# LiZhuoHong/SegLand

Hardware: AMD Instinct MI355X
Metric: 512x512 tiles/sec fwd+bwd PSPNet-POP (higher is better)
Workload: dtype bf16; 1 GPU; PSPNet-POP resnet50 bf16, batch 16/GPU, 512x512, 8 logit channels, train_base.py loop body (fwd+loss+bwd+clip+AdamW x2), 1 x MI355X; global_batch=16, parallelism=dp1

## Files before the change

include/segland_hip_debug.h:

```cpp
#ifndef SEGLAND_HIP_DEBUG_H
#define SEGLAND_HIP_DEBUG_H
#include "segland_hip.h"
#ifdef __cplusplus
extern "C" {
#endif

void sl_debug_reset(void);

void sl_debug_conv_affine(int on);
void sl_debug_conv_p9(int on);
void sl_debug_conv_p9_lean(int on);
void sl_debug_conv_p8_k1(int on);
void sl_debug_conv_ring192(int on);
void sl_debug_conv_ringn64(int on);
void sl_debug_conv_rows_small(int on);
void sl_debug_ppm_fact_walk(int on);
void sl_debug_conv_parity(int on);
void sl_debug_ring_small_k(int k);
void sl_debug_ring64_max_tiles(int tiles);
void sl_debug_wgrad3(int on);
void sl_debug_wgrad_bias(int on);
void sl_debug_wgrad_tr(int on);
void sl_debug_wgrad_pair_min(int rows);
void sl_debug_attn_valu(int v);
void sl_debug_ce_tiled(int on);

void sl_debug_p8_trace(void* buf);
void sl_debug_wgrad_trace(void* buf);
void sl_debug_wgrad3_trace(void* buf);
void sl_debug_attn_trace(void* buf);

int sl_debug_wgrad3_plan(const SlConvDesc* d, int* out);

#ifdef __cplusplus
}
#endif
#endif
```

segland_amd/csrc/api.cpp:

```cpp
#include <stdarg.h>
#include <stdio.h>
#include <mutex>
#include <unordered_map>
#include "common.h"

static thread_local char g_err[512] = "";

void sl_set_error(const char* fmt, ...) {
  va_list ap;
  va_start(ap, fmt);
  vsnprintf(g_err, sizeof(g_err), fmt, ap);
  va_end(ap);
}

extern "C" int sl_version(void) { return 100; }
extern "C" const char* sl_last_error_string(void) { return g_err; }

__attribute__((visibility("hidden"))) int sl_lds_opt_in(const char* name, const void* kernel, size_t lds_bytes) {
  static std::mutex mu;
  static std::unordered_map<const void*, size_t> granted;
  std::lock_guard<std::mutex> lock(mu);
  size_t& have = granted[kernel];
  if (lds_bytes <= have) return 0;
  const hipError_t e = hipFuncSetAttribute(kernel, hipFuncAttributeMaxDynamicSharedMemorySize, (int)lds_bytes);
  if (e != hipSuccess) {
    sl_set_error("%s: opt-in to %zu bytes of dynamic LDS refused: %s", name, lds_bytes, hipGetErrorString(e));
    return (int)e;
  }
  have = lds_bytes;
  return 0;
}

extern "C" int sl_hip_clear_error(void) { return (int)hipGetLastError(); }

#include "../../include/segland_hip_debug.h"
SlDebugState g_sl_debug;
extern "C" void sl_debug_reset(void) { g_sl_debug = SlDebugState(); }
extern "C" void sl_debug_conv_affine(int v) { g_sl_debug.conv_affine = v ? 1 : 0; }
extern "C" void sl_debug_conv_p9(int v) { g_sl_debug.conv_p9 = (v & 1) ? 1 : 0; }
extern "C" void sl_debug_conv_p9_lean(int v) { g_sl_debug.conv_p9_lean = v ? 1 : 0; }
extern "C" void sl_debug_conv_p8_k1(int v) { g_sl_debug.conv_p8_k1 = v ? 1 : 0; }
extern "C" void sl_debug_conv_ring192(int v) { g_sl_debug.conv_ring192 = v ? 1 : 0; }
extern "C" void sl_debug_conv_ringn64(int v) { g_sl_debug.conv_ringn64 = v ? 1 : 0; }
extern "C" void sl_debug_conv_rows_small(int v) { g_sl_debug.conv_rows_small = v ? 1 : 0; }
extern "C" void sl_debug_conv_parity(int v) { g_sl_debug.conv_parity = v ? 1 : 0; }
extern "C" void sl_debug_ppm_fact_walk(int v) { g_sl_debug.ppm_fact_walk = v ? 1 : 0; }
extern "C" void sl_debug_ring64_max_tiles(int v) { g_sl_debug.ring64_max_tiles = v; }
extern "C" void sl_debug_ring_small_k(int v) { g_sl_debug.ring_small_k = v; }
extern "C" void sl_debug_wgrad3(int v) { g_sl_debug.wgrad3 = v ? 1 : 0; }
extern "C" void sl_debug_wgrad_bias(int v) { g_sl_debug.wgrad_bias = v ? 1 : 0; }
extern "C" void sl_debug_wgrad_tr(int v) { g_sl_debug.wgrad_tr = v ? 1 : 0; }
extern "C" void sl_debug_wgrad_pair_min(int rows) { g_sl_debug.wgrad_pair_min_rows = rows; }
extern "C" void sl_debug_attn_valu(int v) { g_sl_debug.attn_valu = v; }
extern "C" void sl_debug_ce_tiled(int v) { g_sl_debug.ce_tiled = v ? 1 : 0; }
extern "C" void sl_debug_p8_trace(void* buf) { g_sl_debug.p8_trace = (unsigned long long*)buf; }
extern "C" void sl_debug_wgrad_trace(void* buf) { g_sl_debug.wgrad_trace = (unsigned long long*)buf; }
extern "C" void sl_debug_wgrad3_trace(void* buf) { g_sl_debug.wgrad3_trace = (unsigned long long*)buf; }
extern "C" void sl_debug_attn_trace(void* buf) { g_sl_debug.attn_trace = (unsigned long long*)buf; }
```

segland_amd/csrc/common.h:

```cpp
#pragma once
#include <hip/hip_runtime.h>
#include <stdint.h>
#include <stdio.h>
#include "../../include/segland_hip.h"

typedef unsigned short bf16_t;

typedef __attribute__((ext_vector_type(8))) __bf16 bf16x8_t;
typedef __attribute__((ext_vector_type(16))) float f32x16_t;
typedef __attribute__((ext_vector_type(4))) float f32x4_t;

__device__ __forceinline__ float bf2f(bf16_t v) { return __uint_as_float(((unsigned)v) << 16); }
__device__ __forceinline__ bf16_t f2bf(float f) {
  return __builtin_bit_cast(bf16_t, (__bf16)f);
}

template <typename T> __device__ __forceinline__ float to_f(T v);
template <> __device__ __forceinline__ float to_f<float>(float v) { return v; }
template <> __device__ __forceinline__ float to_f<bf16_t>(bf16_t v) { return bf2f(v); }
template <typename T> __device__ __forceinline__ T from_f(float v);
template <> __device__ __forceinline__ float from_f<float>(float v) { return v; }
template <> __device__ __forceinline__ bf16_t from_f<bf16_t>(float v) { return f2bf(v); }

template <typename T> struct Vec16 { static constexpr int N = 16 / sizeof(T); };

template <typename T> __device__ __forceinline__ void unpack16(const uint4& v, float* out);
template <> __device__ __forceinline__ void unpack16<float>(const uint4& v, float* out) {
  out[0] = __uint_as_float(v.x); out[1] = __uint_as_float(v.y); out[2] = __uint_as_float(v.z); out[3] = __uint_as_float(v.w);
}
template <> __device__ __forceinline__ void unpack16<bf16_t>(const uint4& v, float* out) {
  out[0] = __uint_as_float(v.x << 16); out[1] = __uint_as_float(v.x & 0xffff0000u);
  out[2] = __uint_as_float(v.y << 16); out[3] = __uint_as_float(v.y & 0xffff0000u);
  out[4] = __uint_as_float(v.z << 16); out[5] = __uint_as_float(v.z & 0xffff0000u);
  out[6] = __uint_as_float(v.w << 16); out[7] = __uint_as_float(v.w & 0xffff0000u);
}
template <typename T> __device__ __forceinline__ uint4 pack16(const float* in);
template <> __device__ __forceinline__ uint4 pack16<float>(const float* in) {
  return make_uint4(__float_as_uint(in[0]), __float_as_uint(in[1]), __float_as_uint(in[2]), __float_as_uint(in[3]));
}
template <> __device__ __forceinline__ uint4 pack16<bf16_t>(const float* in) {
  typedef __attribute__((ext_vector_type(2))) __bf16 bf16x2_t;
  typedef __attribute__((ext_vector_type(2))) float f32x2_t;
  uint4 r;
  r.x = __builtin_bit_cast(unsigned, __builtin_convertvector((f32x2_t){in[0], in[1]}, bf16x2_t));
  r.y = __builtin_bit_cast(unsigned, __builtin_convertvector((f32x2_t){in[2], in[3]}, bf16x2_t));
  r.z = __builtin_bit_cast(unsigned, __builtin_convertvector((f32x2_t){in[4], in[5]}, bf16x2_t));
  r.w = __builtin_bit_cast(unsigned, __builtin_convertvector((f32x2_t){in[6], in[7]}, bf16x2_t));
  return r;
}

__device__ __forceinline__ float sl_erf_as(float x) {
  const float ax = fabsf(x);
  const float t = __builtin_amdgcn_rcpf(fmaf(0.3275911f, ax, 1.f));
  float p = fmaf(1.061405429f, t, -1.453152027f);
  p = fmaf(p, t, 1.421413741f); p = fmaf(p, t, -0.284496736f); p = fmaf(p, t, 0.254829592f);
  const float r = fmaf(-p * t, __expf(-ax * ax), 1.f);
  return copysignf(r, x);
}
template <typename T> __device__ __forceinline__ float sl_gelu(float x) {
  if constexpr (sizeof(T) == 4) return 0.5f * x * (1.f + erff(x * 0.70710678118654752440f));
  else return 0.5f * x * (1.f + sl_erf_as(x * 0.70710678118654752440f));
}

template <typename T> __device__ __forceinline__ float sl_gelu_grad(float x) {
  const float pdf = 0.39894228040143267794f * __expf(-0.5f * x * x);
  float cdf;
  if constexpr (sizeof(T) == 4) cdf = 0.5f * (1.f + erff(x * 0.70710678118654752440f));
  else cdf = 0.5f * (1.f + sl_erf_as(x * 0.70710678118654752440f));
  return cdf + x * pdf;
}

__device__ __forceinline__ float wave_sum(float v) {
#pragma unroll
  for (int o = 32; o > 0; o >>= 1) v += __shfl_xor(v, o, 64);
  return v;
}

void sl_set_error(const char* fmt, ...);

struct SlDebugState {
  int conv_affine = 1;
  int conv_p9 = 1;
  int conv_p9_lean = 1;
  int conv_p8_k1 = 1;
  int conv_ring192 = 1;
  int conv_ringn64 = 1;
  int conv_rows_small = 1;
  int ppm_fact_walk = 1;
  int conv_parity = 1;
  int ring_small_k = 128;
  long long ring64_max_tiles = 256;
  int wgrad3 = 1;
  int wgrad_bias = 1;
  int wgrad_tr = 1;
  long long wgrad_pair_min_rows = 0;
  int attn_valu = -1;
  int ce_tiled = 1;
  unsigned long long* p8_trace = nullptr;
  unsigned long long* wgrad_trace = nullptr;
  unsigned long long* wgrad3_trace = nullptr;
  unsigned long long* attn_trace = nullptr;
};
extern SlDebugState g_sl_debug;
#define SL_REQUIRE(cond, ...)            \
  do {                                   \
    if (!(cond)) {                       \
      sl_set_error(__VA_ARGS__);         \
      return SL_EINVAL;                  \
    }                                    \
  } while (0)
#define SL_TRY(expr)                     \
  do {                                   \
    const int rc__ = (expr);             \
    if (rc__) return rc__;               \
  } while (0)

int sl_lds_opt_in(const char* name, const void* kernel, size_t lds_bytes);

template <typename T> struct sl_as_is { typedef T type; };

template <typename... Args>
static inline int sl_launch(const char* name, void (*kernel)(Args...), dim3 grid, dim3 block, size_t lds_bytes, hipStream_t stream, typename sl_as_is<Args>::type... args) {
  if (lds_bytes > 64 * 1024) SL_TRY(sl_lds_opt_in(name, (const void*)kernel, lds_bytes));
  hipLaunchKernelGGL(kernel, grid, block, lds_bytes, stream, args...);
  const hipError_t e = hipGetLastError();
  if (e != hipSuccess) {
    sl_set_error("%s: %s", name, hipGetErrorString(e));
    return (int)e;
  }
  return 0;
}

template <typename F>
static inline int sl_by_dtype(int dtype, const char* entry, F&& f) {
  if (dtype == SL_BF16) return f(bf16_t());
  if (dtype == SL_F32) return f(float());
  sl_set_error("%s: bad dtype", entry);
  return SL_EINVAL;
}

__host__ __device__ static inline int cdiv(long long a, long long b) { return (int)((a + b - 1) / b); }

template <typename T>
__device__ __forceinline__ void sl_colsum_rows_block(const T* __restrict__ x, long long rows, int C, long long rows_per_block, float* __restrict__ part, int block, float* red) {
  constexpr int V = Vec16<T>::N;
  const int nvec = C / V;
  const int tpr = nvec < 256 ? nvec : 256, rpb = 256 / tpr;
  const int tr = threadIdx.x / tpr, tc = threadIdx.x % tpr;
  const long long r0 = (long long)block * rows_per_block, r1 = r0 + rows_per_block < rows ? r0 + rows_per_block : rows;
  for (int vc = tc; vc < nvec; vc += tpr) {
    float s[V];
#pragma unroll
    for (int k = 0; k < V; ++k) s[k] = 0.f;
    if (tr < rpb) {
      long long r = r0 + tr;
      for (; r + 3 * rpb < r1; r += 4 * rpb) {
        uint4 q[4];
#pragma unroll
        for (int u = 0; u < 4; ++u) q[u] = ((const uint4*)x)[(size_t)(r + u * rpb) * nvec + vc];
#pragma unroll
        for (int u = 0; u < 4; ++u) {
          float v[V];
          unpack16<T>(q[u], v);
#pragma unroll
          for (int k = 0; k < V; ++k) s[k] += v[k];
        }
      }
      for (; r < r1; r += rpb) {
        float v[V];
        unpack16<T>(((const uint4*)x)[(size_t)r * nvec + vc], v);
#pragma unroll
        for (int k = 0; k < V; ++k) s[k] += v[k];
      }
    }
    __syncthreads();
#pragma unroll
    for (int k = 0; k < V; ++k) red[threadIdx.x * V + k] = s[k];
    __syncthreads();
    if (tr == 0) {
#pragma unroll
      for (int k = 0; k < V; ++k) {
        float a = 0.f;
        for (int j = 0; j < rpb; ++j) a += red[(j * tpr + tc) * V + k];
        part[(size_t)block * C + vc * V + k] = a;
      }
    }
  }
}


inline long long sl_colsum_rows_chunk(long long rows, int C, int esize) {
  const int nvec = C * esize / 16, tpr = nvec < 256 ? nvec : 256, rpb = 256 / tpr;
  long long rpblk = (long long)rpb * 16;
  const long long cap = 2048;
  if ((rows + rpblk - 1) / rpblk > cap) rpblk = ((rows + cap - 1) / cap + rpb - 1) / rpb * rpb;
  return rpblk;
}
```

segland_amd/csrc/conv_gemm_sk.hip:

```cpp
#include "conv_gemm_common.h"

namespace {

using slconv::C64_T;
constexpr int C64_PW = C64_T + 2, C64_PITCH = 144;
constexpr int C64_WFRAG = 2 * 36 * 64 * 16;
constexpr int C64_LDS = C64_WFRAG + C64_PW * C64_PW * C64_PITCH + 4 * 2 * 64 * (int)sizeof(float);
__global__ __launch_bounds__(256) void conv_c64k3_kernel(ConvGemmParams p, int ntiles) {
  extern __shared__ __attribute__((aligned(16))) unsigned char smem[];
  uint4* wl = (uint4*)smem;
  unsigned char* patch = smem + C64_WFRAG;
  float* red = (float*)(patch + C64_PW * C64_PW * C64_PITCH);
  const int tid = threadIdx.x, lane = tid & 63, wave = tid >> 6, l31 = lane & 31, fh = lane >> 5;
  const int H = p.Hs, W = p.Ws;
  const int tx = cdiv(W, C64_T), ty = cdiv(H, C64_T);
  const bf16_t* src = (const bf16_t*)p.src1;
  for (int e = tid; e < 2 * 36 * 64; e += 256) {
    const int ln = e & 63, ks = (e >> 6) % 36, nb = (e >> 6) / 36;
    wl[e] = *(const uint4*)((const bf16_t*)p.wt + ((size_t)(nb * 32 + (ln & 31)) * 9 + (ks >> 2)) * 64 + (ks & 3) * 16 + (ln >> 5) * 8);
  }
  constexpr int NCH = C64_PW * C64_PW * 8, CPT = (NCH + 255) / 256;
  uint4 stage[CPT];
  auto fetch = [&](int tile) {
    int blk = tile;
    const int bx = blk % tx; blk /= tx;
    const int by = blk % ty; const int b = blk / ty;
#pragma unroll
    for (int u = 0; u < CPT; ++u) {
      const int e = tid + u * 256;
      uint4 v = make_uint4(0, 0, 0, 0);
      if (e < NCH) {
        const int ch8 = e & 7, pp = e >> 3, py = pp / C64_PW, px = pp - py * C64_PW;
        const int iy = by * C64_T - 1 + py, ix = bx * C64_T - 1 + px;
        if ((unsigned)iy < (unsigned)H && (unsigned)ix < (unsigned)W) v = *(const uint4*)(src + ((size_t)(b * H + iy) * W + ix) * 64 + ch8 * 8);
      }
      stage[u] = v;
    }
  };
  int pbase[2];
#pragma unroll
  for (int rb = 0; rb < 2; ++rb) {
    const int pidx = wave * 64 + rb * 32 + l31;
    pbase[rb] = ((pidx >> 4) * C64_PW + (pidx & 15)) * C64_PITCH + fh * 16;
  }
  if ((int)blockIdx.x < ntiles) fetch(blockIdx.x);
  for (int tile = blockIdx.x; tile < ntiles; tile += gridDim.x) {
    int blk = tile;
    const int bx = blk % tx; blk /= tx;
    const int by = blk % ty; const int b = blk / ty;
#pragma unroll
    for (int u = 0; u < CPT; ++u) {
      const int e = tid + u * 256;
      if (e < NCH) *(uint4*)(patch + (e >> 3) * C64_PITCH + (e & 7) * 16) = stage[u];
    }
    __syncthreads();
    if (tile + (int)gridDim.x < ntiles) fetch(tile + gridDim.x);
    f32x16_t acc[2][2];
#pragma unroll
    for (int rb = 0; rb < 2; ++rb)
#pragma unroll
      for (int nb = 0; nb < 2; ++nb)
#pragma unroll
        for (int r = 0; r < 16; ++r) acc[rb][nb][r] = 0.f;
#pragma unroll 4
    for (int ks = 0; ks < 36; ++ks) {
      int tap = ks >> 2;
      if (p.mode) tap = 8 - tap;
      const int ky = tap / 3, kx = tap - 3 * ky;
      const int toff = (ky * C64_PW + kx) * C64_PITCH + (ks & 3) * 32;
      const uint4 w0 = wl[(0 * 36 + ks) * 64 + lane], w1 = wl[(1 * 36 + ks) * 64 + lane];
#pragma unroll
      for (int rb = 0; rb < 2; ++rb) {
        const uint4 a = *(const uint4*)(patch + pbase[rb] + toff);
        acc[rb][0] = __builtin_amdgcn_mfma_f32_32x32x16_bf16(__builtin_bit_cast(bf16x8_t, w0), __builtin_bit_cast(bf16x8_t, a), acc[rb][0], 0, 0, 0);
        acc[rb][1] = __builtin_amdgcn_mfma_f32_32x32x16_bf16(__builtin_bit_cast(bf16x8_t, w1), __builtin_bit_cast(bf16x8_t, a), acc[rb][1], 0, 0, 0);
      }
    }
    __syncthreads();
    unsigned char* outt = patch;
#pragma unroll
    for (int rb = 0; rb < 2; ++rb) {
      const int pidx = wave * 64 + rb * 32 + l31;
#pragma unroll
      for (int nb = 0; nb < 2; ++nb)
#pragma unroll
        for (int q = 0; q < 4; ++q) {
          uint2 pk;
          pk.x = (unsigned)f2bf(acc[rb][nb][4 * q + 0]) | ((unsigned)f2bf(acc[rb][nb][4 * q + 1]) << 16);
          pk.y = (unsigned)f2bf(acc[rb][nb][4 * q + 2]) | ((unsigned)f2bf(acc[rb][nb][4 * q + 3]) << 16);
          *(uint2*)(outt + pidx * C64_PITCH + (nb * 32 + 8 * q + 4 * fh) * 2) = pk;
        }
    }
    __syncthreads();
    bf16_t* out = (bf16_t*)p.out;
    float sa[8], sq[8];
#pragma unroll
    for (int c = 0; c < 8; ++c) { sa[c] = 0.f; sq[c] = 0.f; }
    if (p.gate) {
      float mu[8], is[8];
#pragma unroll
      for (int c = 0; c < 8; ++c) { mu[c] = p.bn_mean[(tid & 7) * 8 + c]; is[c] = p.bn_invstd[(tid & 7) * 8 + c]; }
      uint4 xv[8]; unsigned bits[8];
#pragma unroll
      for (int u = 0; u < 8; ++u) {
        const int e = tid + u * 256, pidx = e >> 3, ch8 = e & 7;
        const int oy = by * C64_T + (pidx >> 4), ox = bx * C64_T + (pidx & 15);
        const bool in = oy < H && ox < W;
        const size_t pix = in ? (size_t)(b * H + oy) * W + ox : 0;
        xv[u] = *(const uint4*)((const bf16_t*)p.bn_x + pix * 64 + ch8 * 8);
        bits[u] = p.gate[pix * 8 + ch8];
      }
#pragma unroll
      for (int u = 0; u < 8; ++u) {
        const int e = tid + u * 256, pidx = e >> 3, ch8 = e & 7;
        const int oy = by * C64_T + (pidx >> 4), ox = bx * C64_T + (pidx & 15);
        if (oy < H && ox < W) {
          uint4 v = *(const uint4*)(outt + pidx * C64_PITCH + ch8 * 16);
          const unsigned bb = bits[u];
          v.x &= ((unsigned)__builtin_amdgcn_sbfe(bb, 0, 1) & 0xffffu) | ((unsigned)__builtin_amdgcn_sbfe(bb, 1, 1) & 0xffff0000u);
          v.y &= ((unsigned)__builtin_amdgcn_sbfe(bb, 2, 1) & 0xffffu) | ((unsigned)__builtin_amdgcn_sbfe(bb, 3, 1) & 0xffff0000u);
          v.z &= ((unsigned)__builtin_amdgcn_sbfe(bb, 4, 1) & 0xffffu) | ((unsigned)__builtin_amdgcn_sbfe(bb, 5, 1) & 0xffff0000u);
          v.w &= ((unsigned)__builtin_amdgcn_sbfe(bb, 6, 1) & 0xffffu) | ((unsigned)__builtin_amdgcn_sbfe(bb, 7, 1) & 0xffff0000u);
          st16(out + ((size_t)(b * H + oy) * W + ox) * 64 + ch8 * 8, v);
          const unsigned wv[4] = {v.x, v.y, v.z, v.w}, xw[4] = {xv[u].x, xv[u].y, xv[u].z, xv[u].w};
#pragma unroll
          for (int c = 0; c < 4; ++c) {
            const float lo = __uint_as_float(wv[c] << 16), hi = __uint_as_float(wv[c] & 0xffff0000u);
            const float xl = __uint_as_float(xw[c] << 16), xh = __uint_as_float(xw[c] & 0xffff0000u);
            sa[2 * c] += lo; sq[2 * c] += lo * ((xl - mu[2 * c]) * is[2 * c]);
            sa[2 * c + 1] += hi; sq[2 * c + 1] += hi * ((xh - mu[2 * c + 1]) * is[2 * c + 1]);
          }
        }
      }
    } else
#pragma unroll
    for (int u = 0; u < 8; ++u) {
      const int e = tid + u * 256;
      const int pidx = e >> 3, ch8 = e & 7;
      const int oy = by * C64_T + (pidx >> 4), ox = bx * C64_T + (pidx & 15);
      if (oy < H && ox < W) {
        const uint4 v = *(const uint4*)(outt + pidx * C64_PITCH + ch8 * 16);
        st16(out + ((size_t)(b * H + oy) * W + ox) * 64 + ch8 * 8, v);
        if (p.stat_partial) {
          const unsigned wv[4] = {v.x, v.y, v.z, v.w};
#pragma unroll
          for (int c = 0; c < 4; ++c) {
            const float lo = __uint_as_float(wv[c] << 16), hi = __uint_as_float(wv[c] & 0xffff0000u);
            sa[2 * c] += lo; sq[2 * c] += lo * lo; sa[2 * c + 1] += hi; sq[2 * c + 1] += hi * hi;
          }
        }
      }
    }
    if (p.stat_partial) {
#pragma unroll
      for (int c = 0; c < 8; ++c)
#pragma unroll
        for (int o = 8; o < 64; o <<= 1) { sa[c] += __shfl_xor(sa[c], o); sq[c] += __shfl_xor(sq[c], o); }
      if (lane < 8) {
#pragma unroll
        for (int c = 0; c < 8; ++c) { red[(wave * 2 + 0) * 64 + lane * 8 + c] = sa[c]; red[(wave * 2 + 1) * 64 + lane * 8 + c] = sq[c]; }
      }
      __syncthreads();
      if (tid < 128) {
        const int which = tid >> 6, ch = tid & 63;
        p.stat_partial[((size_t)tile * 2 + which) * 64 + ch] = red[(0 * 2 + which) * 64 + ch] + red[(1 * 2 + which) * 64 + ch] + red[(2 * 2 + which) * 64 + ch] + red[(3 * 2 + which) * 64 + ch];
      }
    }
    __syncthreads();
  }
}

}

bool slconv::c64k3_shape(int dtype, int KH, int KW, int stride, int pad, int dil, int Cin, int C1, int Cout, long long M) {
  return dtype == SL_BF16 && KH == 3 && KW == 3 && stride == 1 && pad == 1 && dil == 1 && Cin == 64 && C1 == 64 && Cout == 64 && M >= 65536;
}

int slconv::launch_c64k3(ConvGemmParams& p, hipStream_t st) {
  const int ntiles = p.B * cdiv(p.Hs, C64_T) * cdiv(p.Ws, C64_T);
  return sl_launch("conv_c64k3_kernel", conv_c64k3_kernel, dim3(ntiles < 256 ? ntiles : 256), dim3(256), C64_LDS, st, p, ntiles);
}

namespace {
template <int KS> struct SkGeom {
  static constexpr int RB = KS * 32;
  static constexpr int BSTEP = 64 * RB;
  static constexpr int STG_PITCH = 144, STG_WAVE = 32 * STG_PITCH;
  static constexpr int OFF_STG = 2 * BSTEP, OFF_RED = OFF_STG + 8 * STG_WAVE;
  static constexpr int LDS = OFF_RED + 2 * 8 * 3 * 64 * (int)sizeof(float);
};
template <int KS> __device__ __forceinline__ int sk_swz(int row) { return KS == 16 ? (row & 31) : (KS == 8 ? (row & 15) : ((row >> 1) & 7)); }
__device__ __forceinline__ float sk_sum_8_16_32(float v) {
  typedef __attribute__((ext_vector_type(2))) unsigned u32x2_t;
  v += __int_as_float(__builtin_amdgcn_update_dpp(0, __float_as_int(v), 0x128, 0xf, 0xf, false));
  u32x2_t r = __builtin_amdgcn_permlane16_swap(__float_as_uint(v), __float_as_uint(v), false, false);
  v = __uint_as_float(r.x) + __uint_as_float(r.y);
  r = __builtin_amdgcn_permlane32_swap(__float_as_uint(v), __float_as_uint(v), false, false);
  return __uint_as_float(r.x) + __uint_as_float(r.y);
}

#ifndef SL_SK_ABL
#define SL_SK_ABL 0
#endif
template <int KS, int MODE, bool SKEW>
__global__ __launch_bounds__(512, (KS == 4 && MODE != 5) ? 4 : 2) void conv_gemm_sk_kernel(ConvGemmParams p) {
  using G = SkGeom<KS>;
  using T = bf16_t;
  typedef __attribute__((ext_vector_type(2))) __bf16 bf16x2_t;
  typedef __attribute__((ext_vector_type(2))) float f32x2_t;
  extern __shared__ __attribute__((aligned(16))) unsigned char smem[];
  const int tid = threadIdx.x, lane = tid & 63;
  const int wave = __builtin_amdgcn_readfirstlane(tid >> 6);
  const int grp = wave >> 2;
  const int l31 = lane & 31, fh = lane >> 5;
  const int bm = blockIdx.x;
  const int NS = p.N / 64;
  const unsigned lds_base = __builtin_amdgcn_readfirstlane(lds_addr_of(smem));
  constexpr int NWI = SKEW ? 4 : 8, NI = 2 * KS / NWI, LPR = 2 * KS, RPI = 64 / LPR;
  const int iw = SKEW ? (wave & 3) : wave;
  const bool issuer = !SKEW || grp == 0;
  const unsigned char* bsrc[NI];
#pragma unroll
  for (int j = 0; j < NI; ++j) {
    const int row = (iw * NI + j) * RPI + lane / LPR, pos = lane % LPR;
    bsrc[j] = (const unsigned char*)p.wt + (size_t)row * G::RB + ((pos ^ sk_swz<KS>(row)) << 4);
  }
  auto issueB = [&](int s, int buf) {
#pragma unroll
    for (int j = 0; j < NI; ++j) glds16_asm(bsrc[j] + (size_t)s * G::BSTEP, lds_base + buf * G::BSTEP + (iw * NI + j) * 1024);
  };
  auto colstep = [&](int i) { return i; };
  if (issuer) issueB(colstep(0), 0);
  uint4 a[KS];
  {
    const unsigned char* arow = (const unsigned char*)p.src1 + ((size_t)bm * 256 + wave * 32 + l31) * G::RB + fh * 16;
#pragma unroll
    for (int ks = 0; ks < KS; ++ks) a[ks] = *(const uint4*)(arow + ks * 32);
  }
  int foff[KS];
  {
    const int x = sk_swz<KS>(l31);
#pragma unroll
    for (int ks = 0; ks < KS; ++ks) foff[ks] = l31 * G::RB + (((2 * ks + fh) ^ x) << 4);
  }
  unsigned char* stg = smem + G::OFF_STG + wave * G::STG_WAVE;
  float* red = (float*)(smem + G::OFF_RED);
  const int srow = lane >> 3, sch = lane & 7;
  const size_t orow = (size_t)bm * 256 + wave * 32 + srow;
  long long arow[4];
  if constexpr (MODE == 2 || MODE == 5) {
#pragma unroll
    for (int it = 0; it < 4; ++it) {
      const long long m = (long long)orow + it * 8;
      arow[it] = m;
      if (p.addend_half) {
        const int hw = p.Hd * p.Wd;
        const int b = (int)(m / hw), rem = (int)(m - (long long)b * hw), y = rem / p.Wd, x = rem - y * p.Wd;
        arow[it] = ((y | x) & 1) ? -1 : ((long long)b * (p.Hd >> 1) + (y >> 1)) * (p.Wd >> 1) + (x >> 1);
      }
    }
  }
  uint4 addv[4], cxv[4], cxv2[4];
  float bmu[8], bis[8], bmu2[8], bis2[8];
  const bool dual = MODE == 5 && p.bn_x2 != nullptr;
  const int mpitch = p.N / 8 + 16;
  unsigned char* msk = smem + (MODE == 5 ? G::LDS : G::OFF_RED);
  if ((MODE == 2 && p.addend_mask) || MODE == 5) {
    const int cpr = p.N / 128;
    const unsigned char* src = (MODE == 5 ? p.gate : p.addend_mask) + (size_t)bm * 256 * (p.N / 8);
    for (int e = tid; e < 256 * cpr; e += 512) {
      const int row = e / cpr, c = e - row * cpr;
      *(uint4*)(msk + row * mpitch + c * 16) = *(const uint4*)(src + (size_t)e * 16);
    }
  }

  auto multiply = [&](int i) {
    const int cur = i & 1, s = colstep(i);
    if (issuer && i + 1 < NS) issueB(colstep(i + 1), cur ^ 1);
    if constexpr (MODE == 2 || MODE == 5) {
      const int ncol = s * 64 + sch * 8;
#pragma unroll
      for (int it = 0; it < 4; ++it) addv[it] = (arow[it] >= 0 && !(SL_SK_ABL & 2)) ? *(const uint4*)((const T*)p.addend + arow[it] * p.N + ncol) : make_uint4(0, 0, 0, 0);
      if constexpr (MODE == 5) {
#pragma unroll
        for (int it = 0; it < 4; ++it) cxv[it] = (SL_SK_ABL & 2) ? make_uint4(0, 0, 0, 0) : *(const uint4*)((const T*)p.bn_x + (orow + it * 8) * p.N + ncol);
#pragma unroll
        for (int e = 0; e < 8; ++e) { bmu[e] = p.bn_mean[ncol + e]; bis[e] = p.bn_invstd[ncol + e]; }
        if (dual) {
#pragma unroll
          for (int it = 0; it < 4; ++it) cxv2[it] = *(const uint4*)((const T*)p.bn_x2 + (orow + it * 8) * p.N + ncol);
#pragma unroll
          for (int e = 0; e < 8; ++e) { bmu2[e] = p.bn_mean2[ncol + e]; bis2[e] = p.bn_invstd2[ncol + e]; }
        }
      }
    }
    f32x16_t acc[2];
#pragma unroll
    for (int j = 0; j < 2; ++j)
#pragma unroll
      for (int r = 0; r < 16; ++r) acc[j][r] = 0.f;
    const unsigned char* bb = smem + cur * G::BSTEP;
#pragma unroll
    for (int ks = 0; ks < KS; ++ks) {
      const uint4 b0 = *(const uint4*)(bb + foff[ks]), b1 = *(const uint4*)(bb + 32 * G::RB + foff[ks]);
      if constexpr (!(SL_SK_ABL & 8)) {
      Mma<T>::run(b0, a[ks], acc[0]);
      Mma<T>::run(b1, a[ks], acc[1]);
      } else { acc[0][0] += __uint_as_float(b0.x); acc[1][0] += __uint_as_float(b1.x); }
    }
#pragma unroll
    for (int j = 0; j < 2; ++j)
#pragma unroll
      for (int q = 0; q < 4; ++q) {
        uint2 v;
        v.x = __builtin_bit_cast(unsigned, __builtin_convertvector((f32x2_t){acc[j][4 * q + 0], acc[j][4 * q + 1]}, bf16x2_t));
        v.y = __builtin_bit_cast(unsigned, __builtin_convertvector((f32x2_t){acc[j][4 * q + 2], acc[j][4 * q + 3]}, bf16x2_t));
        *(uint2*)(stg + l31 * G::STG_PITCH + 64 * j + 16 * q + 8 * fh) = v;
      }
  };

  auto store = [&](int i) {
    const int cur = i & 1, s = colstep(i);
    const int ncol = s * 64 + sch * 8;
    wait_vmcnt<0>();
    float sa[8], sq[8], sq2[8];
#pragma unroll
    for (int e = 0; e < 8; ++e) { sa[e] = 0.f; sq[e] = 0.f; sq2[e] = 0.f; }
#pragma unroll
    for (int it = 0; it < 4; ++it) {
      const uint4 raw = *(const uint4*)(stg + (it * 8 + srow) * G::STG_PITCH + sch * 16);
      T* o = (T*)p.out + (orow + it * 8) * p.N + ncol;
      if constexpr (MODE == 1) {
        st16(o, raw);
        if (p.stat_partial) {
          const unsigned w[4] = {raw.x, raw.y, raw.z, raw.w};
#pragma unroll
          for (int c = 0; c < 4; ++c) {
            const float lo = __uint_as_float(w[c] << 16), hi = __uint_as_float(w[c] & 0xffff0000u);
            sa[2 * c] += lo; sq[2 * c] += lo * lo; sa[2 * c + 1] += hi; sq[2 * c + 1] += hi * hi;
          }
        }
      } else {
        uint4 ad = addv[it];
        if (MODE == 2 && p.addend_mask) {
          const unsigned b = msk[(wave * 32 + it * 8 + srow) * mpitch + s * 8 + sch];
          ad.x &= ((unsigned)__builtin_amdgcn_sbfe(b, 0, 1) & 0xffffu) | ((unsigned)__builtin_amdgcn_sbfe(b, 1, 1) & 0xffff0000u);
          ad.y &= ((unsigned)__builtin_amdgcn_sbfe(b, 2, 1) & 0xffffu) | ((unsigned)__builtin_amdgcn_sbfe(b, 3, 1) & 0xffff0000u);
          ad.z &= ((unsigned)__builtin_amdgcn_sbfe(b, 4, 1) & 0xffffu) | ((unsigned)__builtin_amdgcn_sbfe(b, 5, 1) & 0xffff0000u);
          ad.w &= ((unsigned)__builtin_amdgcn_sbfe(b, 6, 1) & 0xffffu) | ((unsigned)__builtin_amdgcn_sbfe(b, 7, 1) & 0xffff0000u);
        }
        const unsigned rw[4] = {raw.x, raw.y, raw.z, raw.w}, aw[4] = {ad.x, ad.y, ad.z, ad.w};
        unsigned ow[4];
#pragma unroll
        for (int c = 0; c < 4; ++c) {
          const f32x2_t v = (f32x2_t){__uint_as_float(rw[c] << 16) + __uint_as_float(aw[c] << 16), __uint_as_float(rw[c] & 0xffff0000u) + __uint_as_float(aw[c] & 0xffff0000u)};
          ow[c] = __builtin_bit_cast(unsigned, __builtin_convertvector(v, bf16x2_t));
        }
        if constexpr (MODE == 5) {
          const unsigned b = msk[(wave * 32 + it * 8 + srow) * mpitch + s * 8 + sch];
          ow[0] &= ((unsigned)__builtin_amdgcn_sbfe(b, 0, 1) & 0xffffu) | ((unsigned)__builtin_amdgcn_sbfe(b, 1, 1) & 0xffff0000u);
          ow[1] &= ((unsigned)__builtin_amdgcn_sbfe(b, 2, 1) & 0xffffu) | ((unsigned)__builtin_amdgcn_sbfe(b, 3, 1) & 0xffff0000u);
          ow[2] &= ((unsigned)__builtin_amdgcn_sbfe(b, 4, 1) & 0xffffu) | ((unsigned)__builtin_amdgcn_sbfe(b, 5, 1) & 0xffff0000u);
          ow[3] &= ((unsigned)__builtin_amdgcn_sbfe(b, 6, 1) & 0xffffu) | ((unsigned)__builtin_amdgcn_sbfe(b, 7, 1) & 0xffff0000u);
          const unsigned xw[4] = {cxv[it].x, cxv[it].y, cxv[it].z, cxv[it].w};
#pragma unroll
          for (int c = 0; c < 4; ++c) {
            if constexpr (SL_SK_ABL & 4) { sa[2 * c] += __uint_as_float(ow[c] ^ xw[c]); continue; }
            const float glo = __uint_as_float(ow[c] << 16), ghi = __uint_as_float(ow[c] & 0xffff0000u);
            const float xlo = __uint_as_float(xw[c] << 16), xhi = __uint_as_float(xw[c] & 0xffff0000u);
            sa[2 * c] += glo; sq[2 * c] += glo * ((xlo - bmu[2 * c]) * bis[2 * c]);
            sa[2 * c + 1] += ghi; sq[2 * c + 1] += ghi * ((xhi - bmu[2 * c + 1]) * bis[2 * c + 1]);
          }
          if (dual) {
            const unsigned yw[4] = {cxv2[it].x, cxv2[it].y, cxv2[it].z, cxv2[it].w};
#pragma unroll
            for (int c = 0; c < 4; ++c) {
              const float glo = __uint_as_float(ow[c] << 16), ghi = __uint_as_float(ow[c] & 0xffff0000u);
              const float ylo = __uint_as_float(yw[c] << 16), yhi = __uint_as_float(yw[c] & 0xffff0000u);
              sq2[2 * c] += glo * ((ylo - bmu2[2 * c]) * bis2[2 * c]);
              sq2[2 * c + 1] += ghi * ((yhi - bmu2[2 * c + 1]) * bis2[2 * c + 1]);
            }
          }
        }
        if constexpr (SL_SK_ABL & 1) { if (ow[0] == 0x12345678u && ow[1] == 0x9abcdef0u) st16(o, make_uint4(ow[0], ow[1], ow[2], ow[3])); }
        else st16(o, make_uint4(ow[0], ow[1], ow[2], ow[3]));
      }
    }
    if ((MODE == 1 || MODE == 5) && p.stat_partial) {
#pragma unroll
      for (int e = 0; e < 8; ++e) { sa[e] = sk_sum_8_16_32(sa[e]); sq[e] = sk_sum_8_16_32(sq[e]); }
      if (dual) {
#pragma unroll
        for (int e = 0; e < 8; ++e) sq2[e] = sk_sum_8_16_32(sq2[e]);
      }
      if (lane < 8) {
        float* r0 = red + ((cur * 8 + wave) * 3) * 64 + sch * 8;
        *(float4*)(r0) = make_float4(sa[0], sa[1], sa[2], sa[3]); *(float4*)(r0 + 4) = make_float4(sa[4], sa[5], sa[6], sa[7]);
        *(float4*)(r0 + 64) = make_float4(sq[0], sq[1], sq[2], sq[3]); *(float4*)(r0 + 68) = make_float4(sq[4], sq[5], sq[6], sq[7]);
        if (dual) { *(float4*)(r0 + 128) = make_float4(sq2[0], sq2[1], sq2[2], sq2[3]); *(float4*)(r0 + 132) = make_float4(sq2[4], sq2[5], sq2[6], sq2[7]); }
      }
    }
  };
  auto finalize = [&](int i, int t0) {
    const int s = colstep(i);
    if ((MODE == 1 || MODE == 5) && p.stat_partial && tid >= t0 && tid < t0 + (dual ? 192 : 128)) {
      const int which = (tid - t0) >> 6, col = tid & 63;
      const float* r0 = red + ((i & 1) * 24 + which) * 64 + col;
      float t = 0.f;
#pragma unroll
      for (int k = 0; k < 8; ++k) t += r0[k * 192];
      if (which < 2) p.stat_partial[((size_t)bm * 2 + which) * p.N + s * 64 + col] = t;
      if (dual && which != 1) p.stat_partial2[((size_t)bm * 2 + (which >> 1)) * p.N + s * 64 + col] = t;
    }
  };

  auto bar = [&]() { asm volatile("s_waitcnt lgkmcnt(0)\n\ts_barrier" ::: "memory"); };
  wait_vmcnt<0>();
  bar();
  if constexpr (!SKEW) {
#pragma unroll 1
    for (int s = 0; s < NS; ++s) {
      multiply(s);
      store(s);
      bar();
      finalize(s, 0);
    }
  } else if (grp == 0) {
#pragma unroll 1
    for (int s = 0; s < NS; ++s) {
      multiply(s);
      bar();
      store(s);
      bar();
    }
    bar();
  } else {
    bar();
#pragma unroll 1
    for (int s = 0; s < NS; ++s) {
      multiply(s);
      bar();
      store(s);
      bar();
      finalize(s, 256);
    }
  }
}

}

bool slconv::sk_shape(int dtype, int KH, int KW, int stride, int pad, int Cin, int C1, int N, long long M) {
  return dtype == SL_BF16 && KH == 1 && KW == 1 && stride == 1 && pad == 0 && C1 == Cin && (Cin == 64 || Cin == 128 || Cin == 256) &&
         N % 64 == 0 && M >= 65536 && M % 256 == 0;
}

namespace {
template <int KS, int MODE, bool SKEW>
int launch_sk_t(ConvGemmParams& p, hipStream_t st) {
  const int lds = MODE == 5 ? SkGeom<KS>::LDS + 256 * (p.N / 8 + 16)
                            : (MODE == 2 && p.addend_mask ? SkGeom<KS>::OFF_RED + 256 * (p.N / 8 + 16) : SkGeom<KS>::LDS);
  return sl_launch("conv_gemm_sk_kernel", conv_gemm_sk_kernel<KS, MODE, SKEW>, dim3(p.M / 256), dim3(512), lds, st, p);
}
template <int MODE, bool SKEW>
int launch_sk_k(ConvGemmParams& p, hipStream_t st) {
  return p.C1 == 256 ? launch_sk_t<16, MODE, SKEW>(p, st) : (p.C1 == 128 ? launch_sk_t<8, MODE, SKEW>(p, st) : launch_sk_t<4, MODE, SKEW>(p, st));
}
}

int slconv::launch_sk(ConvGemmParams& p, hipStream_t st) {
  constexpr int skew = 1;
  p.gridM = p.M / 256; p.gridN = 1;
  if (p.gate) return launch_sk_k<5, false>(p, st);
  if (p.addend) return (skew & 4) ? launch_sk_k<2, true>(p, st) : launch_sk_k<2, false>(p, st);
  return (skew & (p.stat_partial ? 1 : 2)) ? launch_sk_k<1, true>(p, st) : launch_sk_k<1, false>(p, st);
}
```

Before: 699.4 tiles/s.

## Prefetch addend and BN inputs two column steps ahead in sk conv GEMM

```diff
diff --git a/include/segland_hip_debug.h b/include/segland_hip_debug.h
--- a/include/segland_hip_debug.h
+++ b/include/segland_hip_debug.h
@@ -11,6 +11,7 @@
 void sl_debug_conv_p9(int on);
 void sl_debug_conv_p9_lean(int on);
 void sl_debug_conv_p8_k1(int on);
+void sl_debug_conv_sk_ahead(int on);
 void sl_debug_conv_ring192(int on);
 void sl_debug_conv_ringn64(int on);
 void sl_debug_conv_rows_small(int on);
diff --git a/segland_amd/csrc/api.cpp b/segland_amd/csrc/api.cpp
--- a/segland_amd/csrc/api.cpp
+++ b/segland_amd/csrc/api.cpp
@@ -40,6 +40,7 @@
 extern "C" void sl_debug_conv_p9(int v) { g_sl_debug.conv_p9 = (v & 1) ? 1 : 0; }
 extern "C" void sl_debug_conv_p9_lean(int v) { g_sl_debug.conv_p9_lean = v ? 1 : 0; }
 extern "C" void sl_debug_conv_p8_k1(int v) { g_sl_debug.conv_p8_k1 = v ? 1 : 0; }
+extern "C" void sl_debug_conv_sk_ahead(int v) { g_sl_debug.conv_sk_ahead = v ? 1 : 0; }
 extern "C" void sl_debug_conv_ring192(int v) { g_sl_debug.conv_ring192 = v ? 1 : 0; }
 extern "C" void sl_debug_conv_ringn64(int v) { g_sl_debug.conv_ringn64 = v ? 1 : 0; }
 extern "C" void sl_debug_conv_rows_small(int v) { g_sl_debug.conv_rows_small = v ? 1 : 0; }
diff --git a/segland_amd/csrc/common.h b/segland_amd/csrc/common.h
--- a/segland_amd/csrc/common.h
+++ b/segland_amd/csrc/common.h
@@ -83,6 +83,7 @@
   int conv_p9 = 1;
   int conv_p9_lean = 1;
   int conv_p8_k1 = 1;
+  int conv_sk_ahead = 1;
   int conv_ring192 = 1;
   int conv_ringn64 = 1;
   int conv_rows_small = 1;
diff --git a/segland_amd/csrc/conv_gemm_sk.hip b/segland_amd/csrc/conv_gemm_sk.hip
--- a/segland_amd/csrc/conv_gemm_sk.hip
+++ b/segland_amd/csrc/conv_gemm_sk.hip
@@ -199,10 +199,23 @@
   return __uint_as_float(r.x) + __uint_as_float(r.y);
 }
 
+__device__ __forceinline__ void sk_wait_vm0() {
+  asm volatile("" ::: "memory");
+  __builtin_amdgcn_s_waitcnt(0x0f70);
+  asm volatile("" ::: "memory");
+}
+template <int V> struct SkPf { static constexpr int value = V; };
+__device__ __forceinline__ uint4 sk_take(const uint4& v) {
+  uint4 r;
+  asm volatile("v_mov_b32 %0, %4\n\tv_mov_b32 %1, %5\n\tv_mov_b32 %2, %6\n\tv_mov_b32 %3, %7" : "=&v"(r.x), "=&v"(r.y), "=&v"(r.z), "=&v"(r.w) : "v"(v.x), "v"(v.y), "v"(v.z), "v"(v.w));
+  return r;
+}
+__device__ __forceinline__ unsigned sk_fresh(unsigned v) { asm volatile("" : "+v"(v)); return v; }
+
 #ifndef SL_SK_ABL
 #define SL_SK_ABL 0
 #endif
-template <int KS, int MODE, bool SKEW>
+template <int KS, int MODE, bool SKEW, bool AHEAD>
 __global__ __launch_bounds__(512, (KS == 4 && MODE != 5) ? 4 : 2) void conv_gemm_sk_kernel(ConvGemmParams p) {
   using G = SkGeom<KS>;
   using T = bf16_t;
@@ -220,14 +233,17 @@
   const int iw = SKEW ? (wave & 3) : wave;
   const bool issuer = !SKEW || grp == 0;
   const unsigned char* bsrc[NI];
+  unsigned boff[NI];
 #pragma unroll
   for (int j = 0; j < NI; ++j) {
     const int row = (iw * NI + j) * RPI + lane / LPR, pos = lane % LPR;
-    bsrc[j] = (const unsigned char*)p.wt + (size_t)row * G::RB + ((pos ^ sk_swz<KS>(row)) << 4);
+    boff[j] = (unsigned)(row * G::RB + ((pos ^ sk_swz<KS>(row)) << 4));
+    bsrc[j] = (const unsigned char*)p.wt + boff[j];
   }
   auto issueB = [&](int s, int buf) {
 #pragma unroll
-    for (int j = 0; j < NI; ++j) glds16_asm(bsrc[j] + (size_t)s * G::BSTEP, lds_base + buf * G::BSTEP + (iw * NI + j) * 1024);
+    for (int j = 0; j < NI; ++j)
+      glds16_asm((AHEAD ? (const unsigned char*)p.wt + sk_fresh(boff[j]) : bsrc[j]) + (size_t)s * G::BSTEP, lds_base + buf * G::BSTEP + (iw * NI + j) * 1024);
   };
   auto colstep = [&](int i) { return i; };
   if (issuer) issueB(colstep(0), 0);
@@ -237,12 +253,10 @@
 #pragma unroll
     for (int ks = 0; ks < KS; ++ks) a[ks] = *(const uint4*)(arow + ks * 32);
   }
+  const int fswz = sk_swz<KS>(l31);
   int foff[KS];
-  {
-    const int x = sk_swz<KS>(l31);
-#pragma unroll
-    for (int ks = 0; ks < KS; ++ks) foff[ks] = l31 * G::RB + (((2 * ks + fh) ^ x) << 4);
-  }
+#pragma unroll
+  for (int ks = 0; ks < KS; ++ks) foff[ks] = l31 * G::RB + (((2 * ks + fh) ^ fswz) << 4);
   unsigned char* stg = smem + G::OFF_STG + wave * G::STG_WAVE;
   float* red = (float*)(smem + G::OFF_RED);
   const int srow = lane >> 3, sch = lane & 7;
@@ -260,9 +274,26 @@
       }
     }
   }
+  unsigned roff[4], aoff[4];
+#pragma unroll
+  for (int it = 0; it < 4; ++it) {
+    roff[it] = (unsigned)(((orow + it * 8) * p.N + sch * 8) * sizeof(T));
+    aoff[it] = ~0u;
+    if constexpr (MODE == 2 || MODE == 5) { if (arow[it] >= 0) aoff[it] = (unsigned)((arow[it] * p.N + sch * 8) * sizeof(T)); }
+  }
+  auto rowp = [&](const void* base, int it, int s) {
+    if constexpr (AHEAD) return (uint4*)((unsigned char*)base + (size_t)(s * 64 * (int)sizeof(T)) + sk_fresh(roff[it]));
+    else return (uint4*)((T*)base + (orow + it * 8) * p.N + s * 64 + sch * 8);
+  };
+  auto addp = [&](int it, int s) {
+    if constexpr (AHEAD) return (const uint4*)((const unsigned char*)p.addend + (size_t)(s * 64 * (int)sizeof(T)) + sk_fresh(aoff[it]));
+    else return (const uint4*)((const T*)p.addend + arow[it] * p.N + s * 64 + sch * 8);
+  };
+  auto has_add = [&](int it) { return AHEAD ? aoff[it] != ~0u : arow[it] >= 0; };
   uint4 addv[4], cxv[4], cxv2[4];
+  uint4 addvB[4], cxvB[4], cxv2B[4];
   float bmu[8], bis[8], bmu2[8], bis2[8];
-  const bool dual = MODE == 5 && p.bn_x2 != nullptr;
+  const bool dual = !AHEAD && MODE == 5 && p.bn_x2 != nullptr;
   const int mpitch = p.N / 8 + 16;
   unsigned char* msk = smem + (MODE == 5 ? G::LDS : G::OFF_RED);
   if ((MODE == 2 && p.addend_mask) || MODE == 5) {
@@ -273,23 +304,38 @@
       *(uint4*)(msk + row * mpitch + c * 16) = *(const uint4*)(src + (size_t)e * 16);
     }
   }
-
+  const unsigned cf_off = (unsigned)(msk - smem) + 256 * mpitch;
+  const float* cfsrc = nullptr;
+  if constexpr (AHEAD && MODE == 5) cfsrc = ((lane & 16) ? p.bn_invstd : p.bn_mean) + (lane & 15) * 4;
+  auto issueC = [&](int s, int slot) { glds16_asm(cfsrc + s * 64, lds_base + cf_off + slot * 1024); };
+
+  auto fetch = [&](int i, uint4 (&av)[4], uint4 (&cv)[4], uint4 (&cv2)[4]) {
+    const int s = colstep(i);
+#pragma unroll
+    for (int it = 0; it < 4; ++it) av[it] = (has_add(it) && !(SL_SK_ABL & 2)) ? *addp(it, s) : make_uint4(0, 0, 0, 0);
+    if constexpr (MODE == 5) {
+#pragma unroll
+      for (int it = 0; it < 4; ++it) cv[it] = (SL_SK_ABL & 2) ? make_uint4(0, 0, 0, 0) : *rowp((void*)p.bn_x, it, s);
+      if (dual) {
+#pragma unroll
+        for (int it = 0; it < 4; ++it) cv2[it] = *rowp((void*)p.bn_x2, it, s);
+      }
+    }
+  };
   auto multiply = [&](int i) {
     const int cur = i & 1, s = colstep(i);
-    if (issuer && i + 1 < NS) issueB(colstep(i + 1), cur ^ 1);
-    if constexpr (MODE == 2 || MODE == 5) {
-      const int ncol = s * 64 + sch * 8;
-#pragma unroll
-      for (int it = 0; it < 4; ++it) addv[it] = (arow[it] >= 0 && !(SL_SK_ABL & 2)) ? *(const uint4*)((const T*)p.addend + arow[it] * p.N + ncol) : make_uint4(0, 0, 0, 0);
+    if (issuer && i + 1 < NS) {
+      issueB(colstep(i + 1), cur ^ 1);
+      if (AHEAD && MODE == 5 && wave == 0) issueC(colstep(i + 1), cur ^ 1);
+    }
+    if constexpr (!AHEAD && (MODE == 2 || MODE == 5)) {
+      fetch(i, addv, cxv, cxv2);
       if constexpr (MODE == 5) {
-#pragma unroll
-        for (int it = 0; it < 4; ++it) cxv[it] = (SL_SK_ABL & 2) ? make_uint4(0, 0, 0, 0) : *(const uint4*)((const T*)p.bn_x + (orow + it * 8) * p.N + ncol);
+        const int ncol = s * 64 + sch * 8;
 #pragma unroll
         for (int e = 0; e < 8; ++e) { bmu[e] = p.bn_mean[ncol + e]; bis[e] = p.bn_invstd[ncol + e]; }
         if (dual) {
 #pragma unroll
-          for (int it = 0; it < 4; ++it) cxv2[it] = *(const uint4*)((const T*)p.bn_x2 + (orow + it * 8) * p.N + ncol);
-#pragma unroll
           for (int e = 0; e < 8; ++e) { bmu2[e] = p.bn_mean2[ncol + e]; bis2[e] = p.bn_invstd2[ncol + e]; }
         }
       }
@@ -300,9 +346,11 @@
 #pragma unroll
       for (int r = 0; r < 16; ++r) acc[j][r] = 0.f;
     const unsigned char* bb = smem + cur * G::BSTEP;
+    const int x = AHEAD ? (int)sk_fresh(fswz) : fswz;
 #pragma unroll
     for (int ks = 0; ks < KS; ++ks) {
-      const uint4 b0 = *(const uint4*)(bb + foff[ks]), b1 = *(const uint4*)(bb + 32 * G::RB + foff[ks]);
+      const int fo = AHEAD ? l31 * G::RB + (((2 * ks + fh) ^ x) << 4) : foff[ks];
+      const uint4 b0 = *(const uint4*)(bb + fo), b1 = *(const uint4*)(bb + 32 * G::RB + fo);
       if constexpr (!(SL_SK_ABL & 8)) {
       Mma<T>::run(b0, a[ks], acc[0]);
       Mma<T>::run(b1, a[ks], acc[1]);
@@ -319,17 +367,28 @@
       }
   };
 
-  auto store = [&](int i) {
+  auto put = [&](T* o, const uint4& v) {
+    if constexpr ((SL_SK_ABL & 1) && MODE != 1) { if (v.x == 0x12345678u && v.y == 0x9abcdef0u) st16(o, v); }
+    else st16(o, v);
+  };
+  auto store = [&](int i, uint4 (&av)[4], uint4 (&cv)[4], uint4 (&cv2)[4], auto pf) {
     const int cur = i & 1, s = colstep(i);
-    const int ncol = s * 64 + sch * 8;
-    wait_vmcnt<0>();
+    if constexpr (!AHEAD) wait_vmcnt<0>();
+    else if constexpr (MODE == 5) {
+      const float* cf = (const float*)(smem + cf_off + cur * 1024) + sch * 8;
+#pragma unroll
+      for (int h = 0; h < 2; ++h) {
+        *(float4*)(bmu + 4 * h) = *(const float4*)(cf + 4 * h); *(float4*)(bis + 4 * h) = *(const float4*)(cf + 64 + 4 * h);
+      }
+    }
     float sa[8], sq[8], sq2[8];
+    uint4 held[4];
 #pragma unroll
     for (int e = 0; e < 8; ++e) { sa[e] = 0.f; sq[e] = 0.f; sq2[e] = 0.f; }
 #pragma unroll
     for (int it = 0; it < 4; ++it) {
       const uint4 raw = *(const uint4*)(stg + (it * 8 + srow) * G::STG_PITCH + sch * 16);
-      T* o = (T*)p.out + (orow + it * 8) * p.N + ncol;
+      T* o = AHEAD ? nullptr : (T*)rowp(p.out, it, s);
       if constexpr (MODE == 1) {
         st16(o, raw);
         if (p.stat_partial) {
@@ -341,7 +400,7 @@
           }
         }
       } else {
-        uint4 ad = addv[it];
+        uint4 ad = av[it];
         if (MODE == 2 && p.addend_mask) {
           const unsigned b = msk[(wave * 32 + it * 8 + srow) * mpitch + s * 8 + sch];
           ad.x &= ((unsigned)__builtin_amdgcn_sbfe(b, 0, 1) & 0xffffu) | ((unsigned)__builtin_amdgcn_sbfe(b, 1, 1) & 0xffff0000u);
@@ -362,7 +421,7 @@
           ow[1] &= ((unsigned)__builtin_amdgcn_sbfe(b, 2, 1) & 0xffffu) | ((unsigned)__builtin_amdgcn_sbfe(b, 3, 1) & 0xffff0000u);
           ow[2] &= ((unsigned)__builtin_amdgcn_sbfe(b, 4, 1) & 0xffffu) | ((unsigned)__builtin_amdgcn_sbfe(b, 5, 1) & 0xffff0000u);
           ow[3] &= ((unsigned)__builtin_amdgcn_sbfe(b, 6, 1) & 0xffffu) | ((unsigned)__builtin_amdgcn_sbfe(b, 7, 1) & 0xffff0000u);
-          const unsigned xw[4] = {cxv[it].x, cxv[it].y, cxv[it].z, cxv[it].w};
+          const unsigned xw[4] = {cv[it].x, cv[it].y, cv[it].z, cv[it].w};
 #pragma unroll
           for (int c = 0; c < 4; ++c) {
             if constexpr (SL_SK_ABL & 4) { sa[2 * c] += __uint_as_float(ow[c] ^ xw[c]); continue; }
@@ -372,7 +431,7 @@
             sa[2 * c + 1] += ghi; sq[2 * c + 1] += ghi * ((xhi - bmu[2 * c + 1]) * bis[2 * c + 1]);
           }
           if (dual) {
-            const unsigned yw[4] = {cxv2[it].x, cxv2[it].y, cxv2[it].z, cxv2[it].w};
+            const unsigned yw[4] = {cv2[it].x, cv2[it].y, cv2[it].z, cv2[it].w};
 #pragma unroll
             for (int c = 0; c < 4; ++c) {
               const float glo = __uint_as_float(ow[c] << 16), ghi = __uint_as_float(ow[c] & 0xffff0000u);
@@ -382,9 +441,18 @@
             }
           }
         }
-        if constexpr (SL_SK_ABL & 1) { if (ow[0] == 0x12345678u && ow[1] == 0x9abcdef0u) st16(o, make_uint4(ow[0], ow[1], ow[2], ow[3])); }
-        else st16(o, make_uint4(ow[0], ow[1], ow[2], ow[3]));
-      }
+        if constexpr (AHEAD) held[it] = make_uint4(ow[0], ow[1], ow[2], ow[3]); else put(o, make_uint4(ow[0], ow[1], ow[2], ow[3]));
+      }
+    }
+    if constexpr (AHEAD) {
+      sk_wait_vm0();
+#pragma unroll
+      for (int it = 0; it < 4; ++it) put((T*)rowp(p.out, it, s), held[it]);
+      if constexpr (decltype(pf)::value >= 1) {
+#pragma unroll
+        for (int it = 0; it < 4; ++it) { av[it] = sk_take(addvB[it]); if constexpr (MODE == 5) cv[it] = sk_take(cxvB[it]); }
+      }
+      if constexpr (decltype(pf)::value == 2) fetch(i + 2, addvB, cxvB, cxv2B);
     }
     if ((MODE == 1 || MODE == 5) && p.stat_partial) {
 #pragma unroll
@@ -415,13 +483,31 @@
   };
 
   auto bar = [&]() { asm volatile("s_waitcnt lgkmcnt(0)\n\ts_barrier" ::: "memory"); };
-  wait_vmcnt<0>();
+  if constexpr (AHEAD) {
+    if constexpr (MODE == 5) { if (wave == 0) issueC(colstep(0), 0); }
+    fetch(0, addv, cxv, cxv2);
+    if (NS > 1) fetch(1, addvB, cxvB, cxv2B);
+  }
+  if constexpr (AHEAD) sk_wait_vm0(); else wait_vmcnt<0>();
   bar();
-  if constexpr (!SKEW) {
+  if constexpr (AHEAD) {
+    static_assert(!SKEW && MODE != 1, "the AHEAD schedule serves the un-skewed addend forms");
+    auto one = [&](int s, auto& av, auto& cv, auto& cv2, auto pf) {
+      multiply(s);
+      store(s, av, cv, cv2, pf);
+      bar();
+      finalize(s, 0);
+    };
+    int s = 0;
+#pragma unroll 1
+    for (; s + 2 < NS; ++s) one(s, addv, cxv, cxv2, SkPf<2>());
+    if (s + 1 < NS) one(s++, addv, cxv, cxv2, SkPf<1>());
+    one(s, addv, cxv, cxv2, SkPf<0>());
+  } else if constexpr (!SKEW) {
 #pragma unroll 1
     for (int s = 0; s < NS; ++s) {
       multiply(s);
-      store(s);
+      store(s, addv, cxv, cxv2, SkPf<0>());
       bar();
       finalize(s, 0);
     }
@@ -430,7 +516,7 @@
     for (int s = 0; s < NS; ++s) {
       multiply(s);
       bar();
-      store(s);
+      store(s, addv, cxv, cxv2, SkPf<0>());
       bar();
     }
     bar();
@@ -440,7 +526,7 @@
     for (int s = 0; s < NS; ++s) {
       multiply(s);
       bar();
-      store(s);
+      store(s, addv, cxv, cxv2, SkPf<0>());
       bar();
       finalize(s, 256);
     }
@@ -455,11 +541,21 @@
 }
 
 namespace {
+template <int KS, int MODE, bool SKEW, bool AHEAD>
+int launch_sk_a(ConvGemmParams& p, hipStream_t st) {
+  const int lds = MODE == 5 ? SkGeom<KS>::LDS + 256 * (p.N / 8 + 16) + (AHEAD ? 2048 : 0)
+                            : (MODE == 2 && p.addend_mask ? SkGeom<KS>::OFF_RED + 256 * (p.N / 8 + 16) : SkGeom<KS>::LDS);
+  SL_REQUIRE(lds <= 160 * 1024, "conv_gemm_sk_kernel: %d bytes of LDS for N = %d, K = %d", lds, p.N, p.C1);
+  return sl_launch("conv_gemm_sk_kernel", conv_gemm_sk_kernel<KS, MODE, SKEW, AHEAD>, dim3(p.M / 256), dim3(512), lds, st, p);
+}
 template <int KS, int MODE, bool SKEW>
 int launch_sk_t(ConvGemmParams& p, hipStream_t st) {
-  const int lds = MODE == 5 ? SkGeom<KS>::LDS + 256 * (p.N / 8 + 16)
-                            : (MODE == 2 && p.addend_mask ? SkGeom<KS>::OFF_RED + 256 * (p.N / 8 + 16) : SkGeom<KS>::LDS);
-  return sl_launch("conv_gemm_sk_kernel", conv_gemm_sk_kernel<KS, MODE, SKEW>, dim3(p.M / 256), dim3(512), lds, st, p);
+  if constexpr (MODE != 1 && !SKEW) {
+    bool ahead = g_sl_debug.conv_sk_ahead != 0 && (long long)p.M * p.N * (long long)sizeof(bf16_t) < (1ll << 32);
+    if (MODE == 5) ahead = ahead && !p.bn_x2 && (((uintptr_t)p.bn_mean | (uintptr_t)p.bn_invstd) & 15) == 0;
+    if (ahead) return launch_sk_a<KS, MODE, SKEW, true>(p, st);
+  }
+  return launch_sk_a<KS, MODE, SKEW, false>(p, st);
 }
 template <int MODE, bool SKEW>
 int launch_sk_k(ConvGemmParams& p, hipStream_t st) {
@@ -471,6 +567,9 @@
   constexpr int skew = 1;
   p.gridM = p.M / 256; p.gridN = 1;
   if (p.gate) return launch_sk_k<5, false>(p, st);
-  if (p.addend) return (skew & 4) ? launch_sk_k<2, true>(p, st) : launch_sk_k<2, false>(p, st);
+  if (p.addend) {
+    if constexpr (skew & 4) return launch_sk_k<2, true>(p, st);
+    else return launch_sk_k<2, false>(p, st);
+  }
   return (skew & (p.stat_partial ? 1 : 2)) ? launch_sk_k<1, true>(p, st) : launch_sk_k<1, false>(p, st);
 }
```

Result: no change. 701.9 tiles/s, median of 6 (+0.4%).
